# KyleKWKim/LLM-guided-Multimodal-MIL

Hardware: AMD Instinct MI355X
Metric: bags/sec fwd+bwd, N=1024 patches D=512 (higher is better)
Workload: dtype f32; 1 GPU; 32 bags/GPU x 1024 patches x 512 dims, image-only gated-attention MIL fwd+BCE+bwd+allreduce+Adam (BASELINE config 2; x1 GPUs = 32 bags); bags_per_gpu=32, patches=1024, dim=512, global_bags=32, parallelism=dp1, mode=train (dropout 0.5 on patches + 0.25 before the head, in-kernel masks), accum=1, batches_cycled=4, launch=eager

## Files before the change

llm-guided-multimodal-mil_amd/csrc/gate_reduce.h:

```cpp
#pragma once
#include "mil_common.h"
#define GR_NG 384
#define GR_NB 16

__device__ __forceinline__ unsigned short gp_bf16_bits(float v) { return __builtin_bit_cast(unsigned short, (__bf16)v); }
__device__ __forceinline__ float gp_bf16_val(unsigned short b) { return __uint_as_float(((unsigned)b) << 16); }
__device__ __forceinline__ void gp_split3(float v, unsigned short& p0, unsigned short& p1, unsigned short& p2) {
    p0 = gp_bf16_bits(v);
    float r = v - gp_bf16_val(p0);
    r = __builtin_isfinite(r) ? r : 0.f;
    p1 = gp_bf16_bits(r);
    p2 = gp_bf16_bits(r - gp_bf16_val(p1));
}
#define GP_SLICE_ELEMS (3 * 2 * GR_NG * 8)
__host__ __device__ __forceinline__ size_t gp_index(int q, int n, int k) {
    return (size_t)(k >> 4) * GP_SLICE_ELEMS + ((size_t)(q * 2 + ((k >> 3) & 1)) * GR_NG + n) * 8 + (k & 7);
}
__device__ __forceinline__ void gp_store4(unsigned short* __restrict__ Wp, int n, int k, const f32x4 v) {
    ushort4 o[3];
    gp_split3(v[0], o[0].x, o[1].x, o[2].x);
    gp_split3(v[1], o[0].y, o[1].y, o[2].y);
    gp_split3(v[2], o[0].z, o[1].z, o[2].z);
    gp_split3(v[3], o[0].w, o[1].w, o[2].w);
#pragma unroll
    for (int q = 0; q < 3; ++q) *reinterpret_cast<ushort4*>(Wp + gp_index(q, n, k)) = o[q];
}

struct HeadBwdArgs {
    const float* dz;
    const float* M;
    float* dWf;
    float* dbf;
    const float* loss_bag;
    float* loss_out;
    int B, L, C;
    int accumulate;
};
static __device__ __forceinline__ void head_bwd_params_block(const HeadBwdArgs& a, int blk, float (*red)[64],
                                                             const AdamFuse& ad) {
    const int nlb = (a.L + 63) / 64;
    const int lane = threadIdx.x & 63, g = threadIdx.x >> 6;
    if (blk < a.C * nlb) {
        const int c = blk / nlb, j = (blk % nlb) * 64 + lane;
        float v = 0.f;
        if (j < a.L)
            for (int b0 = g; b0 < a.B; b0 += 32) {
                float dzv[8], mv[8];
#pragma unroll
                for (int e = 0; e < 8; ++e) {
                    const int b = min(b0 + 4 * e, a.B - 1);
                    dzv[e] = a.dz[b * a.C + c];
                    mv[e] = a.M[(size_t)b * a.L + j];
                }
#pragma unroll
                for (int e = 0; e < 8; ++e) v = b0 + 4 * e < a.B ? fmaf(dzv[e], mv[e], v) : v;
            }
        red[g][lane] = v;
        __syncthreads();
        if (g == 0 && j < a.L) {
            float* o = a.dWf + (size_t)c * a.L + j;
            float t = red[0][lane] + red[1][lane] + red[2][lane] + red[3][lane];
            if (a.accumulate) t += *o;
            *o = t;
            adam_fused(ad, o, t);
        }
    } else {
        if ((int)threadIdx.x < a.C) {
            const int c = threadIdx.x;
            float v = 0.f;
            for (int b0 = 0; b0 < a.B; b0 += 16) {
                float u[16];
#pragma unroll
                for (int e = 0; e < 16; ++e) u[e] = a.dz[min(b0 + e, a.B - 1) * a.C + c];
#pragma unroll
                for (int e = 0; e < 16; ++e) v += b0 + e < a.B ? u[e] : 0.f;
            }
            if (a.accumulate) v += a.dbf[c];
            a.dbf[c] = v;
            adam_fused(ad, a.dbf + c, v);
        }
        if (a.loss_bag != nullptr && g == 1) {
            float v = 0.f;
            for (int b = lane; b < a.B; b += 64) v += a.loss_bag[b];
            v = wave_allsum(v);
            if (lane == 0) a.loss_out[0] = a.accumulate ? a.loss_out[0] + v : v;
        }
    }
}

static __global__ __launch_bounds__(256) void k_gate_bwd_reduce(const float* __restrict__ part, const float* __restrict__ pbias,
                                                                int S, int SB, int L, float* __restrict__ dWv, float* __restrict__ dbv,
                                                                float* __restrict__ dWu, float* __restrict__ dbu,
                                                                float* __restrict__ dw, float* __restrict__ db, int accumulate,
                                                                float wscale, int head_first = 1 << 30,
                                                                HeadBwdArgs head = HeadBwdArgs{}, AdamFuse ad_in = AdamFuse{},
// ... 126 lines not shown
```

llm-guided-multimodal-mil_amd/csrc/gated_pool.hip:

```cpp
#include "mil_internal.h"
#include "philox.h"
#include "gate_reduce.h"
#include <type_traits>

#define GF_TM 128
#define GF_BK 32
#define GF_NG 384

typedef __attribute__((address_space(3))) void lds_void;
__device__ __forceinline__ unsigned bitmask1(unsigned m, int b) { return (unsigned)__builtin_amdgcn_sbfe((int)m, b, 1); }
__device__ __forceinline__ float keep_if(float v, unsigned m, int b) {
    return __uint_as_float(__float_as_uint(v) & bitmask1(m, b));
}
template <bool DROP>
__global__ __launch_bounds__(512) void k_gate_fwd(const float* __restrict__ x, const float* __restrict__ Wv,
                                                       const float* __restrict__ bv, const float* __restrict__ Wu,
                                                       const float* __restrict__ bu, const float* __restrict__ wvec,
                                                       const float* __restrict__ battn, float* __restrict__ scores,
                                                       float* __restrict__ gates, int R, int L,
                                                       const uint32_t* __restrict__ xbits, float xscale) {
    __shared__ __attribute__((aligned(16))) float smem[2 * (GF_TM + GF_NG) * 32];
    float* xs = smem;
    float* ws = smem + 2 * GF_TM * 32;
    const int tid = threadIdx.x, lane = tid & 63, wave = tid >> 6;
// ... 1090 lines not shown
#pragma unroll
                    for (int i = 0; i < 16; ++i) acc[a][b][i] += fold[((a * 2 + b) * 16 + i) * 64 + lane];
        }
    }

    {
        __syncthreads();
        if (grp == 0) {
            float* tw = smem + wave * (64 * 64);
#pragma unroll
            for (int a = 0; a < 2; ++a)
#pragma unroll
                for (int b = 0; b < 2; ++b)
#pragma unroll
                    for (int i = 0; i < 16; ++i) tw[(32 * a + mfma32_row(i, h)) * 64 + 32 * b + r] = acc[a][b][i];
            float* pt = part + ((size_t)s * GF_NG + 128 * m + 64 * wi) * L + j0 + 64 * wj;
            const int c4 = lane & 15, rr = lane >> 4;
#pragma unroll
            for (int pass = 0; pass < 16; ++pass) {
                const int row = 4 * pass + rr;
                const f32x4 v = *reinterpret_cast<const f32x4*>(tw + row * 64 + 4 * c4);
                *reinterpret_cast<f32x4*>(pt + (size_t)row * L + 4 * c4) = v;
            }
        }
    }
#else
    {
        __syncthreads();
        float* tw = smem + wave * (64 * 64);
#pragma unroll
        for (int a = 0; a < 2; ++a)
#pragma unroll
            for (int b = 0; b < 2; ++b)
#pragma unroll
                for (int i = 0; i < 16; ++i) tw[(32 * a + mfma32_row(i, h)) * 64 + 32 * b + r] = acc[a][b][i];
        if (KG == 2) __syncthreads();
        float* pt = part + ((size_t)s * GF_NG + 128 * m + 64 * wi) * L + j0 + 64 * wj;
        const int c4 = lane & 15, rr = lane >> 4;
        const float* t0 = smem_all + wave * (64 * 64);
        const float* t1 = smem_all + (2 * 2 * GB_BKR * 128) + wave * (64 * 64);
        constexpr int NP = 16 / KG;
#pragma unroll
        for (int pass = 0; pass < NP; ++pass) {
            const int row = 4 * (pass + NP * grp) + rr;
            f32x4 v = *reinterpret_cast<const f32x4*>(t0 + row * 64 + 4 * c4);
            if (KG == 2) v += *reinterpret_cast<const f32x4*>(t1 + row * 64 + 4 * c4);
            *reinterpret_cast<f32x4*>(pt + (size_t)row * L + 4 * c4) = v;
        }
    }
#endif

    if (jt == 0) {
        float* redf = smem_all;
        const int arow_all = arow + 16 * grp;
        __syncthreads();
#pragma unroll
        for (int e = 0; e < 4; ++e) {
            redf[(arow_all * 3 + 0) * 64 + 4 * ad4 + e] = acc_bv[e];
            redf[(arow_all * 3 + 1) * 64 + 4 * ad4 + e] = acc_bu[e];
            redf[(arow_all * 3 + 2) * 64 + 4 * ad4 + e] = acc_w[e];
        }
        __syncthreads();
        if (grp == 0 && tid < 192) {
            const int which = tid / 64, d = tid % 64;
            float v = 0.f;
#pragma unroll
            for (int g = 0; g < 16 * KG; ++g) v += redf[(g * 3 + which) * 64 + d];
            pbias[((size_t)s * 4 + which) * 192 + 64 * m + d] = v;
        }
        if (m == 0) {
            __syncthreads();
            redf[threadIdx.x] = acc_ds;
            __syncthreads();
            if (threadIdx.x == 0) {
                float v = 0.f;
                for (int g = 0; g < 256 * KG; g += 16) v += redf[g];
                pbias[((size_t)s * 4 + 3) * 192] = v;
            }
        }
    }
}



template <bool DROP>
__global__ __launch_bounds__(512) void k_gate_bwd_dw2(const float* __restrict__ x, const float* __restrict__ gates,
                                                      const float* __restrict__ ds, const float* __restrict__ wvec,
                                                      float* __restrict__ part, float* __restrict__ pbias, int R, int L,
                                                      int KC, int NJ, const uint32_t* __restrict__ xbits,
                                                      const int32_t* __restrict__ rows_dev) {
    __shared__ __attribute__((aligned(16))) float smem_all[2 * 2 * 2 * GB_BKR * 128];
    if (rows_dev != nullptr) R = min(R, __builtin_amdgcn_readfirstlane(rows_dev[0]));
    const int grp = __builtin_amdgcn_readfirstlane((int)(threadIdx.x >> 8));
    float* smem = smem_all + grp * (2 * 2 * GB_BKR * 128);
    const int tid = threadIdx.x & 255, lane = tid & 63, wave = tid >> 6;
    const int wi = wave >> 1, wj = wave & 1;
    const int r = lane & 31, h = lane >> 5;
    int bid = blockIdx.x;
    {
        const int nwg = gridDim.x, q = nwg >> 3, rem = nwg & 7, xcd = bid & 7;
        bid = (xcd < rem ? xcd * (q + 1) : rem * (q + 1) + (xcd - rem) * q) + (bid >> 3);
    }
    const int jt = bid % NJ, m = (bid / NJ) % 3, s = bid / (3 * NJ);
    const int j0 = jt * 128;
    const int cbeg = min(s * KC, R), cend = min(R, cbeg + KC);
    const int half = ((cend - cbeg + 2 * GB_BKR - 1) / (2 * GB_BKR)) * GB_BKR;
    const int rbeg = min(cend, cbeg + grp * half), rend = min(cend, rbeg + half);
    const int nloop = (min(half, cend - cbeg) + GB_BKR - 1) / GB_BKR;

    const int xrow = tid >> 5, xc4 = tid & 31;
    const int arow = tid >> 4, ad4 = tid & 15;
    const int LW = L >> 5;
    int vx[4], vm[4], vg[2], vd[2];
#pragma unroll
    for (int i = 0; i < 4; ++i) {
        vx[i] = ((xrow + 8 * i) * L + j0 + 4 * xc4) * 4;
        vm[i] = ((xrow + 8 * i) * LW + ((j0 + 4 * xc4) >> 5)) * 4;
    }
#pragma unroll
    for (int i = 0; i < 2; ++i) {
        vg[i] = ((arow + 16 * i) * GF_NG + 64 * m + 4 * ad4) * 4;
        vd[i] = (arow + 16 * i) * 4;
    }
    const f32x4 w4 = *reinterpret_cast<const f32x4*>(wvec + 64 * m + 4 * ad4);
    auto blkpos = [](int c) { return (c & 31) | ((c & 32) << 1) | ((c & 64) >> 1); };
    float* const ab = smem;
    float* const xb = smem + 2 * GB_BKR * 128;
    float* const xw = xb + xrow * 128 + blkpos(4 * xc4);
    float* const aw = ab + arow * 128 + blkpos(4 * ad4);
    const float* const ap = ab + h * 128 + 32 * wi + r;
    const float* const bp = xb + h * 128 + 32 * wj + r;

    u32x4_t rx[4], rv[2], ru[2];
    unsigned rm[4] = {0, 0, 0, 0};
    float rds[2];
    f32x4 rt[2];
    f32x4 acc_bv = {0, 0, 0, 0}, acc_bu = {0, 0, 0, 0}, acc_w = {0, 0, 0, 0};
    float acc_ds = 0.f;

    auto x_srd = [&](int row0) {
        return __builtin_amdgcn_make_buffer_rsrc((void*)(x + (size_t)row0 * L), 0, max(rend - row0, 0) * L * 4, MIL_SRD_FLAGS);
    };
    auto g_srd = [&](int row0) {
        return __builtin_amdgcn_make_buffer_rsrc((void*)(gates + (size_t)row0 * GF_NG), 0, max(rend - row0, 0) * GF_NG * 4,
                                                 MIL_SRD_FLAGS);
    };
    auto d_srd = [&](int row0) {
        return __builtin_amdgcn_make_buffer_rsrc((void*)(ds + row0), 0, max(rend - row0, 0) * 4, MIL_SRD_FLAGS);
    };
    auto m_srd = [&](int row0) {
        return __builtin_amdgcn_make_buffer_rsrc((void*)(xbits + (size_t)row0 * LW), 0, max(rend - row0, 0) * LW * 4,
                                                 MIL_SRD_FLAGS);
    };
    auto xload = [&](int i, int row0) {
        rx[i] = __builtin_amdgcn_raw_buffer_load_b128(x_srd(row0), vx[i], 0, 0);
        if (DROP) rm[i] = __builtin_amdgcn_raw_buffer_load_b32(m_srd(row0), vm[i], 0, 0);
    };
    auto aload = [&](int i, int row0) {
        const __amdgpu_buffer_rsrc_t g = g_srd(row0);
        rv[i] = __builtin_amdgcn_raw_buffer_load_b128(g, vg[i], 0, 0);
        ru[i] = __builtin_amdgcn_raw_buffer_load_b128(g, vg[i] + 192 * 4, 0, 0);
        rds[i] = __uint_as_float(__builtin_amdgcn_raw_buffer_load_b32(d_srd(row0), vd[i], 0, 0));
    };
    auto xwrite = [&](int i, int buf) {
        f32x4 v = __builtin_bit_cast(f32x4, rx[i]);
        if (DROP) {
// ... 13 lines not shown
    auto awrite_u = [&](int i, int buf, bool pub) {
        const f32x4 t = rt[i], u = __builtin_bit_cast(f32x4, ru[i]);
        const f32x4 pu = t - t * u;
        *reinterpret_cast<f32x4*>(aw + (buf * GB_BKR + 16 * i) * 128 + 32) = pu;
        if (pub) {
            const f32x4 v = __builtin_bit_cast(f32x4, rv[i]);
            acc_bv += (rds[i] * w4) * u - t * v;
            acc_bu += pu;
            acc_w += (rds[i] * v) * u;
            if (ad4 == 0) acc_ds += rds[i];
        }
    };

    f32x16 acc[2][2];
#pragma unroll
    for (int a = 0; a < 2; ++a)
#pragma unroll
        for (int b = 0; b < 2; ++b)
#pragma unroll
            for (int i = 0; i < 16; ++i) acc[a][b][i] = 0.f;

#pragma unroll
    for (int i = 0; i < 4; ++i) xload(i, rbeg);
#pragma unroll
    for (int i = 0; i < 2; ++i) aload(i, rbeg);
#pragma unroll
    for (int i = 0; i < 4; ++i) xwrite(i, 0);
#pragma unroll
    for (int i = 0; i < 2; ++i) { awrite_v(i, 0); awrite_u(i, 0, jt == 0); }
#pragma unroll
    for (int i = 0; i < 4; ++i) xload(i, rbeg + GB_BKR);
#pragma unroll
    for (int i = 0; i < 2; ++i) aload(i, rbeg + GB_BKR);
    __syncthreads();

    auto slice = [&](int sl, auto buf_c) {
        constexpr int buf = decltype(buf_c)::value;
        const int row2 = rbeg + (sl + 2) * GB_BKR;
        const bool pub = ((sl + 1) % NJ) == jt;
        const float* apb = ap + buf * GB_BKR * 128;
        const float* bpb = bp + buf * GB_BKR * 128;
        float fa[2][2], fb[2][2];
        fa[0][0] = apb[0]; fa[0][1] = apb[64]; fb[0][0] = bpb[0]; fb[0][1] = bpb[64];
#pragma unroll
        for (int ks = 0; ks < GB_BKR / 2; ++ks) {
            const int q = ks & 1;
            acc[0][0] = __builtin_amdgcn_mfma_f32_32x32x2f32(fa[q][0], fb[q][0], acc[0][0], 0, 0, 0);
            __builtin_amdgcn_sched_barrier(0);
            if (ks + 1 < GB_BKR / 2) {
                fa[q ^ 1][0] = apb[(ks + 1) * 256]; fa[q ^ 1][1] = apb[(ks + 1) * 256 + 64];
                fb[q ^ 1][0] = bpb[(ks + 1) * 256]; fb[q ^ 1][1] = bpb[(ks + 1) * 256 + 64];
            }
            __builtin_amdgcn_sched_barrier(0);
            acc[0][1] = __builtin_amdgcn_mfma_f32_32x32x2f32(fa[q][0], fb[q][1], acc[0][1], 0, 0, 0);
            __builtin_amdgcn_sched_barrier(0);
            if (ks >= 1 && ks <= 4) xwrite(ks - 1, buf ^ 1);
            if (ks == 5) awrite_v(0, buf ^ 1);
            if (ks == 6) awrite_u(0, buf ^ 1, pub);
            if (ks == 7) awrite_v(1, buf ^ 1);
            if (ks == 8) awrite_u(1, buf ^ 1, pub);
            __builtin_amdgcn_sched_barrier(0);
            acc[1][0] = __builtin_amdgcn_mfma_f32_32x32x2f32(fa[q][1], fb[q][0], acc[1][0], 0, 0, 0);
            __builtin_amdgcn_sched_barrier(0);
            if (ks >= 1 && ks <= 4) xload(ks - 1, row2);
            if (ks == 6) aload(0, row2);
            if (ks == 8) aload(1, row2);
            __builtin_amdgcn_sched_barrier(0);
            acc[1][1] = __builtin_amdgcn_mfma_f32_32x32x2f32(fa[q][1], fb[q][1], acc[1][1], 0, 0, 0);
            __builtin_amdgcn_sched_barrier(0);
        }
    };
    int sl = 0;
    for (; sl + 1 < nloop; sl += 2) {
        slice(sl, std::integral_constant<int, 0>{});
        __syncthreads();
        slice(sl + 1, std::integral_constant<int, 1>{});
        __syncthreads();
    }
    if (sl < nloop) {
        slice(sl, std::integral_constant<int, 0>{});
        __syncthreads();
    }

    {
        float* tw = smem + wave * (64 * 64);
#pragma unroll
        for (int a = 0; a < 2; ++a)
#pragma unroll
            for (int b = 0; b < 2; ++b)
#pragma unroll
                for (int i = 0; i < 16; ++i) tw[(32 * a + mfma32_row(i, h)) * 64 + 32 * b + r] = acc[a][b][i];
        __syncthreads();
        float* pt = part + ((size_t)s * GF_NG + 128 * m + 64 * wi) * L + j0 + 64 * wj;
        const int c4 = lane & 15, rr = lane >> 4;
        const float* t0 = smem_all + wave * (64 * 64);
        const float* t1 = smem_all + (2 * 2 * GB_BKR * 128) + wave * (64 * 64);
#pragma unroll
        for (int pass = 0; pass < 8; ++pass) {
            const int row = 4 * (pass + 8 * grp) + rr;
            const f32x4 v = *reinterpret_cast<const f32x4*>(t0 + row * 64 + 4 * c4) +
                            *reinterpret_cast<const f32x4*>(t1 + row * 64 + 4 * c4);
            *reinterpret_cast<f32x4*>(pt + (size_t)row * L + 4 * c4) = v;
        }
    }

    {
        float* redf = smem_all;
        const int arow_all = arow + 16 * grp;
        __syncthreads();
#pragma unroll
        for (int e = 0; e < 4; ++e) {
            redf[(arow_all * 3 + 0) * 64 + 4 * ad4 + e] = acc_bv[e];
            redf[(arow_all * 3 + 1) * 64 + 4 * ad4 + e] = acc_bu[e];
            redf[(arow_all * 3 + 2) * 64 + 4 * ad4 + e] = acc_w[e];
        }
        __syncthreads();
        float* pb = pbias + ((size_t)s * NJ + jt) * 4 * 192;
        if (threadIdx.x < 192) {
            const int which = threadIdx.x / 64, d = threadIdx.x % 64;
            float v = 0.f;
#pragma unroll
            for (int g = 0; g < 32; ++g) v += redf[(g * 3 + which) * 64 + d];
            pb[which * 192 + 64 * m + d] = v;
        }
        if (m == 0) {
            __syncthreads();
            redf[threadIdx.x] = acc_ds;
            __syncthreads();
            if (threadIdx.x == 0) {
                float v = 0.f;
                for (int g = 0; g < 512; g += 16) v += redf[g];
                pb[3 * 192] = v;
            }
        }
    }
}

#include "gate_reduce.h"

extern "C" int mil_abi_version(void) { return 8; }

#define GS_TM 32
#define GS_LS 36
#define GS_THREADS 768
template <bool DROP, int RT>
__global__ __launch_bounds__(GS_THREADS) void k_gate_fwd_r32(const float* __restrict__ x, const float* __restrict__ Wv,
                                                             const float* __restrict__ bv, const float* __restrict__ Wu,
                                                             const float* __restrict__ bu, const float* __restrict__ wvec,
                                                             const float* __restrict__ battn, float* __restrict__ scores,
                                                             float* __restrict__ gates, int R, int L,
                                                             const uint32_t* __restrict__ xbits, float xscale,
                                                             const int32_t* __restrict__ rows_dev) {
    constexpr int TM = GS_TM * RT;
    if (rows_dev != nullptr && (int)(blockIdx.x * TM) >= __builtin_amdgcn_readfirstlane(rows_dev[0])) return;
    __shared__ __attribute__((aligned(16))) float smem[2 * (TM + GF_NG) * GS_LS];
    float* xs = smem;
    float* ws = smem + 2 * TM * GS_LS;
    const int tid = threadIdx.x, lane = tid & 63, wave = tid >> 6;
    const int c = wave >> 1, isu = wave & 1;
    const int r = lane & 31, h = lane >> 5;
    const int row0 = blockIdx.x * TM;
    const float* wsrc[4];
    int wdst[4];
#pragma unroll
    for (int i = 0; i < 4; ++i) {
        const int id = tid + GS_THREADS * i, wrow = id >> 3, ch = id & 7;
        wsrc[i] = (wrow < 192 ? Wv + (size_t)wrow * L : Wu + (size_t)(wrow - 192) * L) + 4 * ch;
        wdst[i] = wrow * GS_LS + 4 * ch;
    }
    const int xrow = (tid % (256 * RT)) >> 3, xch = tid & 7;
    const float* xsrc = x + (size_t)min(row0 + xrow, R - 1) * L + 4 * xch;
    const uint32_t* msrc = DROP ? xbits + (size_t)min(row0 + xrow, R - 1) * (L / 32) : nullptr;
    const int xdst = xrow * GS_LS + 4 * xch;
    f32x4 wreg[2][4], xreg[2];
    unsigned mreg[2] = {0, 0};
    auto gload = [&](int set, int k0) {
#pragma unroll
        for (int i = 0; i < 4; ++i) wreg[set][i] = *reinterpret_cast<const f32x4*>(wsrc[i] + k0);
        xreg[set] = *reinterpret_cast<const f32x4*>(xsrc + k0);
        if (DROP) mreg[set] = msrc[k0 >> 5];
    };
    auto swrite = [&](int set, int buf) {
#pragma unroll
        for (int i = 0; i < 4; ++i) *reinterpret_cast<f32x4*>(ws + buf * GF_NG * GS_LS + wdst[i]) = wreg[set][i];
        if (tid < 256 * RT) {
            f32x4 v = xreg[set];
            if (DROP) {
                const unsigned m = mreg[set] >> (4 * xch);
#pragma unroll
                for (int e = 0; e < 4; ++e) v[e] = keep_if(v[e], m, e) * xscale;
            }
            *reinterpret_cast<f32x4*>(xs + buf * TM * GS_LS + xdst) = v;
        }
    };
    f32x16 acc[RT];
#pragma unroll
    for (int q = 0; q < RT; ++q)
#pragma unroll
        for (int i = 0; i < 16; ++i) acc[q][i] = 0.f;
    const int nslice = L / GF_BK;
    gload(0, 0);
    swrite(0, 0);
    gload(1, min(1, nslice - 1) * GF_BK);
    gload(0, min(2, nslice - 1) * GF_BK);
    __syncthreads();
    auto iteration = [&](int s, int set) {
        const int buf = s & 1;
        const float* xa = xs + buf * TM * GS_LS + r * GS_LS + 4 * h;
        const float* wb = ws + buf * GF_NG * GS_LS + (192 * isu + 32 * c + r) * GS_LS + 4 * h;
        f32x4 fa[RT][4], fb[4];
#pragma unroll
        for (int t = 0; t < 4; ++t) {
#pragma unroll
            for (int q = 0; q < RT; ++q) fa[q][t] = *reinterpret_cast<const f32x4*>(xa + q * GS_TM * GS_LS + 8 * t);
            fb[t] = *reinterpret_cast<const f32x4*>(wb + 8 * t);
        }
        swrite(set, buf ^ 1);
        gload(set, min(s + 3, nslice - 1) * GF_BK);
// ... 340 lines not shown
    MIL_CHECK_LAUNCH();
    return MIL_OK;
}

extern "C" int mil_attn_pool_partial_h(const float* x, const float* scores, const int32_t* tile_map, int T, int L,
                                       float* partials, const float* Wf, int C, float* hrow, const uint32_t* xbits,
                                       float xscale, const uint32_t* mbits, float mscale, void* stream) {
    if (!x || !scores || !tile_map || !partials || !Wf || !hrow) return MIL_EINVAL;
    if (L <= 0 || (L % 256) != 0 || L > 1024 || T < 0 || C <= 0 || C > 4) return MIL_EINVAL;
    return launch_pool_partial(x, scores, tile_map, T, L, partials, Wf, C, hrow, (hipStream_t)stream, xbits, xscale, mbits,
                               mscale);
}

extern "C" int mil_attn_pool_bwd_from_h(const float* scores, const float* lse, const float* hrow, const float* dz,
                                        const float* cdot, const int32_t* tile_map, int T, int C, float* ds, void* stream) {
    if (!scores || !lse || !hrow || !dz || !cdot || !tile_map || !ds || T < 0 || C <= 0 || C > 4) return MIL_EINVAL;
    if (T == 0) return MIL_OK;
    hipLaunchKernelGGL(k_pool_ds_from_h, dim3((T + 7) / 8), dim3(256), 0, (hipStream_t)stream, scores, lse, hrow, dz, cdot,
                       tile_map, T, C, ds);
    MIL_CHECK_LAUNCH();
    return MIL_OK;
}

extern "C" int mil_attn_pool_partial(const float* x, const float* scores, const int32_t* tile_map, int T, int L,
                                     float* partials, const uint32_t* xbits, float xscale, void* stream) {
    if (!x || !scores || !tile_map || !partials) return MIL_EINVAL;
    if (L <= 0 || (L % 256) != 0 || L > 1024 || T < 0) return MIL_EINVAL;
    return launch_pool_partial(x, scores, tile_map, T, L, partials, nullptr, 0, nullptr, (hipStream_t)stream, xbits, xscale);
}

extern "C" int mil_attn_pool_fwd(const float* x, const float* scores, const int32_t* tile_map,
                                 const int32_t* bag_tile_off, int T, int B, int L, float* partials, float* M,
                                 float* lse, const uint32_t* xbits, float xscale, void* stream) {
    if (!x || !scores || !tile_map || !bag_tile_off || !partials || !M || !lse) return MIL_EINVAL;
    if (L <= 0 || (L % 256) != 0 || L > 1024 || B < 0 || T < 0) return MIL_EINVAL;
    hipStream_t st = (hipStream_t)stream;
    const int rc = launch_pool_partial(x, scores, tile_map, T, L, partials, nullptr, 0, nullptr, st, xbits, xscale);
    if (rc != MIL_OK) return rc;
    if (B > 0) {
        hipLaunchKernelGGL(k_pool_merge, dim3(B, L / 128), dim3(256), 0, st, partials, bag_tile_off, M, lse, L, T);
        MIL_CHECK_LAUNCH();
    }
    return MIL_OK;
}

extern "C" int mil_attn_pool_bwd(const float* x, const float* scores, const float* lse, const float* dM,
                                 const float* cdot, const int32_t* tile_map, int T, int L, float* ds, float* dx,
                                 const uint32_t* xbits, float xscale, void* stream) {
    if (!x || !scores || !lse || !dM || !cdot || !tile_map || !ds) return MIL_EINVAL;
    if (L <= 0 || (L % 256) != 0 || L > 1024 || T < 0) return MIL_EINVAL;
    if (T == 0) return MIL_OK;
    hipStream_t st = (hipStream_t)stream;
    switch (L / 256) {
        case 1: hipLaunchKernelGGL(k_pool_bwd_ds<1>, dim3(T), dim3(256), 0, st, x, scores, lse, dM, cdot, tile_map, ds, dx, L, xbits, xscale); break;
        case 2: hipLaunchKernelGGL(k_pool_bwd_ds<2>, dim3(T), dim3(256), 0, st, x, scores, lse, dM, cdot, tile_map, ds, dx, L, xbits, xscale); break;
        case 3: hipLaunchKernelGGL(k_pool_bwd_ds<3>, dim3(T), dim3(256), 0, st, x, scores, lse, dM, cdot, tile_map, ds, dx, L, xbits, xscale); break;
        default: hipLaunchKernelGGL(k_pool_bwd_ds<4>, dim3(T), dim3(256), 0, st, x, scores, lse, dM, cdot, tile_map, ds, dx, L, xbits, xscale); break;
    }
    MIL_CHECK_LAUNCH();
    return MIL_OK;
}

template <bool XB16>
static void launch_gate_bwd_dw(const void* x, const float* gates, const float* ds, const float* w, float* part, float* pbias,
                               int R, int L, int kc, int NJ, int S, int kg, const uint32_t* xbits, hipStream_t st,
                               const int32_t* rows_dev = nullptr) {
    const dim3 grid(S * 3 * NJ);
    if (kg == 2) {
        if (xbits) hipLaunchKernelGGL((k_gate_bwd_dw<XB16, 2, true>), grid, dim3(512), 0, st, x, gates, ds, w, part, pbias, R, L, kc, NJ, xbits, rows_dev);
        else hipLaunchKernelGGL((k_gate_bwd_dw<XB16, 2, false>), grid, dim3(512), 0, st, x, gates, ds, w, part, pbias, R, L, kc, NJ, xbits, rows_dev);
    } else {
        if (xbits) hipLaunchKernelGGL((k_gate_bwd_dw<XB16, 1, true>), grid, dim3(256), 0, st, x, gates, ds, w, part, pbias, R, L, kc, NJ, xbits, rows_dev);
        else hipLaunchKernelGGL((k_gate_bwd_dw<XB16, 1, false>), grid, dim3(256), 0, st, x, gates, ds, w, part, pbias, R, L, kc, NJ, xbits, rows_dev);
    }
}

static inline size_t gate_bwd_ws_floats(int S, int L) { return (size_t)S * GF_NG * L + (size_t)S * (L / 128) * 4 * 192; }

extern "C" size_t mil_gate_bwd_workspace_floats(int R, int L) {
    if (R <= 0 || L <= 0 || (L % 128) != 0) return 0;
    return gate_bwd_ws_floats(gate_dw_plan(R, L, MIL_NUM_CU).S, L);
}

static int gate_bwd_partials_impl(const float* x, const float* gates, const float* ds, const float* w, int R, int L,
                                  int D, float* workspace, size_t workspace_floats, const uint32_t* xbits,
                                  const int32_t* rows_dev, void* stream) {
    if (!x || !gates || !ds || !w || !workspace) return MIL_EINVAL;
    if (D != MIL_GATE_D || L <= 0 || (L % 128) != 0 || R <= 0) return MIL_EINVAL;
    const GateDwPlan p = gate_dw_plan(R, L, MIL_NUM_CU);
    const int S = p.S, kc = p.kc, NJ = L / 128;
    if (workspace_floats < gate_bwd_ws_floats(S, L)) return MIL_ENOSPC;
    float* pb = workspace + (size_t)S * GF_NG * L;
    if (p.dw == MIL_ROUTE_DW2) {
        if (xbits)
            hipLaunchKernelGGL(k_gate_bwd_dw2<true>, dim3(S * 3 * NJ), dim3(512), 0, (hipStream_t)stream, x, gates, ds, w, workspace, pb,
                               R, L, kc, NJ, xbits, rows_dev);
        else
            hipLaunchKernelGGL(k_gate_bwd_dw2<false>, dim3(S * 3 * NJ), dim3(512), 0, (hipStream_t)stream, x, gates, ds, w, workspace, pb,
                               R, L, kc, NJ, xbits, rows_dev);
        MIL_CHECK_LAUNCH();
        return MIL_OK;
    }
    launch_gate_bwd_dw<false>((const void*)x, gates, ds, w, workspace, pb, R, L, kc, NJ, S, p.dw == MIL_ROUTE_DW_KG2 ? 2 : 1, xbits,
                              (hipStream_t)stream, rows_dev);
    MIL_CHECK_LAUNCH();
    return MIL_OK;
}

extern "C" int mil_gate_bwd_partials(const float* x, const float* gates, const float* ds, const float* w, int R, int L,
                                     int D, float* workspace, size_t workspace_floats, const uint32_t* xbits,
                                     void* stream) {
    return gate_bwd_partials_impl(x, gates, ds, w, R, L, D, workspace, workspace_floats, xbits, nullptr, stream);
}
extern "C" int mil_gate_bwd_partials_rows(const float* x, const float* gates, const float* ds, const float* w, int R, int L,
                                          int D, float* workspace, size_t workspace_floats, const uint32_t* xbits,
                                          const int32_t* rows_dev, void* stream) {
    return gate_bwd_partials_impl(x, gates, ds, w, R, L, D, workspace, workspace_floats, xbits, rows_dev, stream);
}

static int gate_bwd_fold(const float* workspace, int R, int L, float* dWv, float* dbv, float* dWu, float* dbu, float* dw, float* db,
                         int accumulate, float wscale, void* stream, const HeadBwdArgs* head = nullptr,
                         const AdamFuse* ad = nullptr, uint16_t* Wp = nullptr) {
    const GateDwPlan p = gate_dw_plan(R, L, MIL_NUM_CU);
    return launch_gate_bwd_reduce(workspace, workspace + (size_t)p.S * GF_NG * L, p.S, p.dw == MIL_ROUTE_DW2 ? p.S * (L / 128) : p.S,
                                  L, dWv, dbv, dWu, dbu, dw, db, accumulate, wscale, (hipStream_t)stream, head, ad, nullptr,
                                  nullptr, Wp);
}

extern "C" int mil_gate_bwd_reduce(const float* workspace, int R, int L, float* dWv, float* dbv, float* dWu, float* dbu,
                                   float* dw, float* db, int accumulate, float xscale, void* stream) {
    if (!workspace || !dWv || !dbv || !dWu || !dbu || !dw || !db) return MIL_EINVAL;
    if (L <= 0 || (L % 128) != 0 || R <= 0) return MIL_EINVAL;
    return gate_bwd_fold(workspace, R, L, dWv, dbv, dWu, dbu, dw, db, accumulate, xscale, stream);
}

extern "C" int mil_gate_bwd_params_head(const float* x, const float* gates, const float* ds, const float* w, int R, int L,
                                        int D, float* workspace, size_t workspace_floats, float* dWv, float* dbv,
                                        float* dWu, float* dbu, float* dw, float* db, int accumulate, const float* dz,
                                        const float* M, float* dWf, float* dbf, int B, int C, const float* loss_bag,
                                        float* loss_out, const uint32_t* xbits, float xscale, void* stream) {
    if (!dWv || !dbv || !dWu || !dbu || !dw || !db || !dz || !M || !dWf || !dbf) return MIL_EINVAL;
    if (B <= 0 || C <= 0 || C > 32 || (loss_bag && !loss_out)) return MIL_EINVAL;
    const int rc = mil_gate_bwd_partials(x, gates, ds, w, R, L, D, workspace, workspace_floats, xbits, stream);
    if (rc != MIL_OK) return rc;
    const HeadBwdArgs head{dz, M, dWf, dbf, loss_bag, loss_out, B, L, C, accumulate};
    return gate_bwd_fold(workspace, R, L, dWv, dbv, dWu, dbu, dw, db, accumulate, xbits ? xscale : 1.0f, stream, &head);
}

extern "C" int mil_gate_bwd_reduce_head(const float* workspace, int R, int L, float* dWv, float* dbv, float* dWu, float* dbu,
                                        float* dw, float* db, int accumulate, float xscale, const float* dz, const float* M,
                                        float* dWf, float* dbf, int B, int C, const float* loss_bag, float* loss_out,
                                        void* stream) {
    if (!workspace || !dWv || !dbv || !dWu || !dbu || !dw || !db || !dz || !M || !dWf || !dbf) return MIL_EINVAL;
    if (L <= 0 || (L % 128) != 0 || R <= 0 || B <= 0 || C <= 0 || C > 32 || (loss_bag && !loss_out)) return MIL_EINVAL;
    const HeadBwdArgs head{dz, M, dWf, dbf, loss_bag, loss_out, B, L, C, accumulate};
    return gate_bwd_fold(workspace, R, L, dWv, dbv, dWu, dbu, dw, db, accumulate, xscale, stream, &head);
}

extern "C" int mil_gate_bwd_reduce_head_adam(const float* workspace, int R, int L, float* dWv, float* dbv, float* dWu,
                                             float* dbu, float* dw, float* db, int accumulate, float xscale, const float* dz,
                                             const float* M, float* dWf, float* dbf, int B, int C, const float* loss_bag,
                                             float* loss_out, float* param_flat, const float* grad_flat, size_t n_param,
                                             float* exp_avg, float* exp_avg_sq, int step, float lr, float beta1, float beta2,
                                             float eps, float weight_decay, float grad_scale, void* stream) {
    return gate_bwd_reduce_head_adam_impl(workspace, R, L, dWv, dbv, dWu, dbu, dw, db, accumulate, xscale, dz, M, dWf, dbf, B, C,
                                          loss_bag, loss_out, param_flat, grad_flat, n_param, exp_avg, exp_avg_sq, step, nullptr,
                                          lr, nullptr, beta1, beta2, eps, weight_decay, grad_scale, stream);
}

int gate_bwd_reduce_head_adam_impl(const float* workspace, int R, int L, float* dWv, float* dbv, float* dWu, float* dbu,
                                   float* dw, float* db, int accumulate, float xscale, const float* dz, const float* M,
                                   float* dWf, float* dbf, int B, int C, const float* loss_bag, float* loss_out,
                                   float* param_flat, const float* grad_flat, size_t n_param, float* exp_avg,
                                   float* exp_avg_sq, int step, const int* step_dev, float lr, const float* lr_dev, float beta1,
                                   float beta2, float eps, float weight_decay, float grad_scale, void* stream, int* done,
// ... 316 lines not shown
```

llm-guided-multimodal-mil_amd/csrc/gated_pool_bf16.hip:

```cpp
#include <stdlib.h>

#include "mil_internal.h"
#include "gate_reduce.h"

typedef __bf16 bf16x8 __attribute__((ext_vector_type(8)));
typedef unsigned short u16x8 __attribute__((ext_vector_type(8)));
typedef unsigned short u16;

__device__ __forceinline__ float bf16_to_f32(u16 v) { return __uint_as_float(((unsigned)v) << 16); }

__device__ __forceinline__ u16x8 keep_bf16x8(const u16x8 v, unsigned bits8) {
    typedef unsigned int u32x4k __attribute__((ext_vector_type(4)));
    u32x4k d = __builtin_bit_cast(u32x4k, v);
#pragma unroll
    for (int e = 0; e < 4; ++e) {
        const unsigned m2 = (bits8 >> (2 * e)) & 3u;
        const unsigned y = (m2 | (m2 << 15)) & 0x00010001u;
        d[e] &= (y << 16) - y;
    }
    return __builtin_bit_cast(u16x8, d);
}
__device__ __forceinline__ u16x8 keep_bf16x8_b(const u16x8 v, unsigned bits8) {
    typedef unsigned int u32x4k __attribute__((ext_vector_type(4)));
    u32x4k d = __builtin_bit_cast(u32x4k, v);
// ... 645 lines not shown
            head_row(c, wf);
#pragma unroll
            for (int i = 0; i < MIL_POOL_TILE / 4; ++i) {
                float d = 0.f;
#pragma unroll
                for (int q = 0; q < NQ; ++q)
#pragma unroll
                    for (int e = 0; e < 8; ++e) d += bf16_to_f32(v[i][q][e]) * wf[q][e];
                d = wave_allsum(d);
                const int rr = wave + 4 * i;
                if (lane == 0 && rr < nrows_) hrow[(size_t)(row0 + rr) * C + c] = d;
            }
        }
    }
    if (wave > 0) {
#pragma unroll
        for (int q = 0; q < NQ; ++q)
#pragma unroll
            for (int e = 0; e < 8; ++e) red[((wave - 1) * NQ + q) * 512 + 8 * lane + e] = acc[q][e];
    }
    __syncthreads();
    if (wave == 0) {
        float* out = partials + (size_t)t * L;
#pragma unroll
        for (int q = 0; q < NQ; ++q)
#pragma unroll
            for (int e = 0; e < 8; ++e) {
                float s = acc[q][e];
#pragma unroll
                for (int w = 0; w < 3; ++w) s += red[(w * NQ + q) * 512 + 8 * lane + e];
                out[512 * q + 8 * lane + e] = s;
            }
        if (lane == 0) {
            float* ml = partials + (size_t)gridDim.x * L + 2 * t;
            ml[0] = ml_lds[0];
            ml[1] = ml_lds[1];
        }
    }
}

template <int NQ>
__global__ __launch_bounds__(256) void k_pool_bwd_ds_bf16(const u16* __restrict__ x, const float* __restrict__ scores,
                                                          const float* __restrict__ lse, const float* __restrict__ dM,
                                                          const float* __restrict__ cdot,
                                                          const int32_t* __restrict__ tile_map, float* __restrict__ ds,
                                                          int L, const uint32_t* __restrict__ xbits, float xscale) {
    const int tid = threadIdx.x, lane = tid & 63, wave = tid >> 6;
    const int t = blockIdx.x;
    const int bag = tile_map[4 * t], row0 = tile_map[4 * t + 1], nrows = tile_map[4 * t + 2];
    float g[NQ][8];
#pragma unroll
    for (int q = 0; q < NQ; ++q)
#pragma unroll
        for (int e = 0; e < 8; ++e) g[q][e] = dM[(size_t)bag * L + 512 * q + 8 * lane + e];
    const float lse_b = lse[bag], c_b = cdot[bag];
    u16x8 v[MIL_POOL_TILE / 4][NQ];
    float sc[MIL_POOL_TILE / 4];
#pragma unroll
    for (int i = 0; i < MIL_POOL_TILE / 4; ++i) {
        const size_t row = (size_t)(row0 + min(wave + 4 * i, nrows - 1));
        const u16* xr = x + row * L + 8 * lane;
#pragma unroll
        for (int q = 0; q < NQ; ++q) v[i][q] = *reinterpret_cast<const u16x8*>(xr + 512 * q);
        if (xbits != nullptr) {
            const uint32_t* mr = xbits + row * (L >> 5) + (lane >> 2);
#pragma unroll
            for (int q = 0; q < NQ; ++q) v[i][q] = keep_bf16x8(v[i][q], mr[16 * q] >> (8 * (lane & 3)));
        }
        sc[i] = scores[row];
    }
#pragma unroll
    for (int i = 0; i < MIL_POOL_TILE / 4; ++i) {
        const int rr = wave + 4 * i;
        float dot = 0.f;
#pragma unroll
        for (int q = 0; q < NQ; ++q)
#pragma unroll
            for (int e = 0; e < 8; ++e) dot += bf16_to_f32(v[i][q][e]) * g[q][e];
        dot = wave_allsum(dot);
        if (rr < nrows && lane == 0) ds[row0 + rr] = expf(sc[i] - lse_b) * (dot * xscale - c_b);
    }
}

#define WB_S 160
typedef short s16x4 __attribute__((ext_vector_type(4)));
typedef __attribute__((address_space(3))) s16x4 lds_s16x4;

__device__ __forceinline__ u16x8 tr_frag(const u16* img, int row, int col) {
    const s16x4 lo = __builtin_amdgcn_ds_read_tr16_b64_v4i16((lds_s16x4*)(img + row * WB_S + col));
    const s16x4 hi = __builtin_amdgcn_ds_read_tr16_b64_v4i16((lds_s16x4*)(img + (row + 4) * WB_S + col));
    u16x8 f;
    f[0] = lo[0]; f[1] = lo[1]; f[2] = lo[2]; f[3] = lo[3];
    f[4] = hi[0]; f[5] = hi[1]; f[6] = hi[2]; f[7] = hi[3];
    return f;
}

__device__ __forceinline__ ushort4 pack_bf16x4(const f32x4 v) {
    ushort4 o;
    o.x = __builtin_bit_cast(u16, (__bf16)v[0]);
    o.y = __builtin_bit_cast(u16, (__bf16)v[1]);
    o.z = __builtin_bit_cast(u16, (__bf16)v[2]);
    o.w = __builtin_bit_cast(u16, (__bf16)v[3]);
    return o;
}

#define WB_BKR 64
#if !defined(WB_SETS)
#define WB_SETS 1
#endif
template <bool DROP>
__global__ __launch_bounds__(256) __attribute__((amdgpu_waves_per_eu(1, 1))) void k_gate_bwd_dw_bf16(const u16* __restrict__ x, const u16* __restrict__ gates,
                                                          const float* __restrict__ ds, const float* __restrict__ wvec,
                                                          float* __restrict__ part, float* __restrict__ pbias, int R, int L,
                                                          int KC, int NJ, const uint32_t* __restrict__ xbits) {
    __shared__ __attribute__((aligned(16))) u16 smem[2 * (WB_BKR * WB_S + WB_BKR * 2 * WB_S)];
    constexpr int ASZ = WB_BKR * WB_S, BSZ = WB_BKR * 2 * WB_S;
    u16* ab = smem;
    u16* xb = smem + 2 * ASZ;
    const int tid = threadIdx.x, lane = tid & 63, wave = tid >> 6;
    const int wi = wave >> 1, wj = wave & 1;
    const int h = lane >> 5;
    const int tq = (lane & 15) >> 2, tp = lane & 3, tg = (lane >> 4) & 1;
    int bid = blockIdx.x;
    {
        const int nwg = gridDim.x, q = nwg >> 3, rem = nwg & 7, xcd = bid & 7;
        bid = (xcd < rem ? xcd * (q + 1) : rem * (q + 1) + (xcd - rem) * q) + (bid >> 3);
    }
    const int jt = bid % NJ, m = (bid / NJ) % 3, s = bid / (3 * NJ);
    const int j0 = jt * 256;
    const int rbeg = s * KC, rend = min(R, rbeg + KC);
    const int nslice = (rend - rbeg + WB_BKR - 1) / WB_BKR;

    const int xrow = tid >> 5, xc = tid & 31;
    const int arow = tid >> 4, ad4 = tid & 15;
    const f32x4 w4 = *reinterpret_cast<const f32x4*>(wvec + 64 * m + 4 * ad4);
    u16x8 rx[WB_SETS][8];
    ushort4 hv[WB_SETS][4], hu[WB_SETS][4];
    float rds[WB_SETS][4], rmask[WB_SETS][4];
    f32x4 acc_bv = {0, 0, 0, 0}, acc_bu = {0, 0, 0, 0}, acc_w = {0, 0, 0, 0};
    float acc_ds = 0.f;

    unsigned rxm[WB_SETS][DROP ? 8 : 1];
    auto xload = [&](int z, int i, int rs) {
        const int gr = min(rs + xrow + 8 * i, rend - 1);
#if !defined(WB_ABL_NOX)
        rx[z][i] = *reinterpret_cast<const u16x8*>(x + (size_t)gr * L + j0 + 8 * xc);
#else
        asm volatile("" : "+v"(rx[z][i]) : "v"(gr));
#endif
        if (DROP) rxm[z][i] = xbits[(size_t)gr * (L >> 5) + ((j0 + 8 * xc) >> 5)];
    };
    auto xwrite = [&](int z, int i, int buf) {
        u16* dst = xb + buf * BSZ + (xc >> 4) * ASZ + (xrow + 8 * i) * WB_S + 8 * (xc & 15);
#if !defined(WB_ABL_NOXW)
        *reinterpret_cast<u16x8*>(dst) = DROP ? keep_bf16x8_b(rx[z][i], rxm[z][i] >> (8 * (xc & 3))) : rx[z][i];
#else
        asm volatile("" ::"v"(rx[z][i]), "v"(dst));
#endif
    };
    auto aload = [&](int z, int i, int rs, bool live) {
        const int gr = rs + arow + 16 * i;
        const int gc = min(gr, rend - 1);
        const u16* gp = gates + (size_t)gc * HB_NG + 64 * m + 4 * ad4;
#if !defined(WB_ABL_NOG)
        hv[z][i] = *reinterpret_cast<const ushort4*>(gp);
        hu[z][i] = *reinterpret_cast<const ushort4*>(gp + 192);
        rds[z][i] = ds[gc];
#else
        asm volatile("" : "+v"(hv[z][i]), "+v"(hu[z][i]), "+v"(rds[z][i]) : "v"(gp));
#endif
        rmask[z][i] = (live && gr < rend) ? 1.f : 0.f;
    };
    auto awrite = [&](int z, int i, int buf) {
#if defined(WB_ABL_NOAW)
        asm volatile("" ::"v"(hv[z][i]), "v"(hu[z][i]), "v"(rds[z][i]), "v"(buf));
        return;
#endif
        const f32x4 v = {bf16_to_f32(hv[z][i].x), bf16_to_f32(hv[z][i].y), bf16_to_f32(hv[z][i].z), bf16_to_f32(hv[z][i].w)};
// ... 532 lines not shown
```

Measured before the change: 153,100 bags/s.

## Add bf16x3-split MFMA path for gate backward weight-gradient kernel

Adds a new dW2 kernel that splits each fp32 operand of x and the gate-derived factors into three bf16 pieces, stages them in LDS and computes the product with 32x32x16 bf16 MFMAs. It uses six cross-piece products per slice, dropping the smallest terms, instead of the slow fp32 32x32x2 MFMA. The new kernel double-buffers with register prefetch interleaved between MFMAs. It is enabled by default via an environment switch. It trades exact fp32 accumulation for a near-fp32 emulation and adds split/convert ALU work and LDS traffic. The tile store and bias-sum epilogue are factored into shared helpers, and tr_frag moves into a common header.

```diff
diff --git a/llm-guided-multimodal-mil_amd/csrc/gate_reduce.h b/llm-guided-multimodal-mil_amd/csrc/gate_reduce.h
--- a/llm-guided-multimodal-mil_amd/csrc/gate_reduce.h
+++ b/llm-guided-multimodal-mil_amd/csrc/gate_reduce.h
@@ -11,6 +11,18 @@
     r = __builtin_isfinite(r) ? r : 0.f;
     p1 = gp_bf16_bits(r);
     p2 = gp_bf16_bits(r - gp_bf16_val(p1));
+}
+#define WB_S 160
+typedef short s16x4 __attribute__((ext_vector_type(4)));
+typedef __attribute__((address_space(3))) s16x4 lds_s16x4;
+typedef unsigned short gp_u16x8 __attribute__((ext_vector_type(8)));
+__device__ __forceinline__ gp_u16x8 tr_frag(const unsigned short* img, int row, int col) {
+    const s16x4 lo = __builtin_amdgcn_ds_read_tr16_b64_v4i16((lds_s16x4*)(img + row * WB_S + col));
+    const s16x4 hi = __builtin_amdgcn_ds_read_tr16_b64_v4i16((lds_s16x4*)(img + (row + 4) * WB_S + col));
+    gp_u16x8 f;
+    f[0] = lo[0]; f[1] = lo[1]; f[2] = lo[2]; f[3] = lo[3];
+    f[4] = hi[0]; f[5] = hi[1]; f[6] = hi[2]; f[7] = hi[3];
+    return f;
 }
 #define GP_SLICE_ELEMS (3 * 2 * GR_NG * 8)
 __host__ __device__ __forceinline__ size_t gp_index(int q, int n, int k) {
diff --git a/llm-guided-multimodal-mil_amd/csrc/gated_pool.hip b/llm-guided-multimodal-mil_amd/csrc/gated_pool.hip
--- a/llm-guided-multimodal-mil_amd/csrc/gated_pool.hip
+++ b/llm-guided-multimodal-mil_amd/csrc/gated_pool.hip
@@ -1196,6 +1196,61 @@
 }
 
 
+__device__ __forceinline__ void dw2_store_tile(float* smem_all, const f32x16 (&acc)[2][2], float* __restrict__ part, int s, int m,
+                                               int L, int j0, int grp, int wave, int lane) {
+    const int wi = wave >> 1, wj = wave & 1, r = lane & 31, h = lane >> 5;
+    float* tw = smem_all + grp * (2 * 2 * GB_BKR * 128) + wave * (64 * 64);
+#pragma unroll
+    for (int a = 0; a < 2; ++a)
+#pragma unroll
+        for (int b = 0; b < 2; ++b)
+#pragma unroll
+            for (int i = 0; i < 16; ++i) tw[(32 * a + mfma32_row(i, h)) * 64 + 32 * b + r] = acc[a][b][i];
+    __syncthreads();
+    float* pt = part + ((size_t)s * GF_NG + 128 * m + 64 * wi) * L + j0 + 64 * wj;
+    const int c4 = lane & 15, rr = lane >> 4;
+    const float* t0 = smem_all + wave * (64 * 64);
+    const float* t1 = smem_all + (2 * 2 * GB_BKR * 128) + wave * (64 * 64);
+#pragma unroll
+    for (int pass = 0; pass < 8; ++pass) {
+        const int row = 4 * (pass + 8 * grp) + rr;
+        const f32x4 v = *reinterpret_cast<const f32x4*>(t0 + row * 64 + 4 * c4) +
+                        *reinterpret_cast<const f32x4*>(t1 + row * 64 + 4 * c4);
+        *reinterpret_cast<f32x4*>(pt + (size_t)row * L + 4 * c4) = v;
+    }
+}
+__device__ __forceinline__ void dw2_publish_sums(float* smem_all, float* __restrict__ pbias, int s, int NJ, int jt, int m,
+                                                 int arow_all, int ad4, const f32x4 acc_bv, const f32x4 acc_bu,
+                                                 const f32x4 acc_w, float acc_ds) {
+    float* redf = smem_all;
+    __syncthreads();
+#pragma unroll
+    for (int e = 0; e < 4; ++e) {
+        redf[(arow_all * 3 + 0) * 64 + 4 * ad4 + e] = acc_bv[e];
+        redf[(arow_all * 3 + 1) * 64 + 4 * ad4 + e] = acc_bu[e];
+        redf[(arow_all * 3 + 2) * 64 + 4 * ad4 + e] = acc_w[e];
+    }
+    __syncthreads();
+    float* pb = pbias + ((size_t)s * NJ + jt) * 4 * 192;
+    if (threadIdx.x < 192) {
+        const int which = threadIdx.x / 64, d = threadIdx.x % 64;
+        float v = 0.f;
+#pragma unroll
+        for (int g = 0; g < 32; ++g) v += redf[(g * 3 + which) * 64 + d];
+        pb[which * 192 + 64 * m + d] = v;
+    }
+    if (m == 0) {
+        __syncthreads();
+        redf[threadIdx.x] = acc_ds;
+        __syncthreads();
+        if (threadIdx.x == 0) {
+            float v = 0.f;
+            for (int g = 0; g < 512; g += 16) v += redf[g];
+            pb[3 * 192] = v;
+        }
+    }
+}
+
 
 template <bool DROP>
 __global__ __launch_bounds__(512) void k_gate_bwd_dw2(const float* __restrict__ x, const float* __restrict__ gates,
@@ -1375,58 +1430,189 @@
         __syncthreads();
     }
 
+    dw2_store_tile(smem_all, acc, part, s, m, L, j0, grp, wave, lane);
+    dw2_publish_sums(smem_all, pbias, s, NJ, jt, m, arow + 16 * grp, ad4, acc_bv, acc_bu, acc_w, acc_ds);
+}
+
+#define GQ_PSZ (GB_BKR * WB_S)
+#define GQ_BUF (6 * GQ_PSZ)
+template <bool DROP>
+__global__ __launch_bounds__(512) void k_gate_bwd_dw2_pieces(const float* __restrict__ x, const float* __restrict__ gates,
+                                                             const float* __restrict__ ds, const float* __restrict__ wvec,
+                                                             float* __restrict__ part, float* __restrict__ pbias, int R, int L,
+                                                             int KC, int NJ, const uint32_t* __restrict__ xbits,
+                                                             const int32_t* __restrict__ rows_dev) {
+    __shared__ __attribute__((aligned(16))) float smem_all[2 * 2 * 2 * GB_BKR * 128];
+    static_assert(2 * GQ_BUF * 2 <= (int)sizeof(smem_all), "stages exceed the LDS image");
+    unsigned short* const img = reinterpret_cast<unsigned short*>(smem_all);
+    if (rows_dev != nullptr) R = min(R, __builtin_amdgcn_readfirstlane(rows_dev[0]));
+    const int grp = __builtin_amdgcn_readfirstlane((int)(threadIdx.x >> 8));
+    const int T = threadIdx.x, tid = T & 255, lane = tid & 63, wave = tid >> 6;
+    const int wi = wave >> 1, wj = wave & 1;
+    const int h = lane >> 5;
+    const int tq = (lane & 15) >> 2, tp = lane & 3, tg = (lane >> 4) & 1;
+    int bid = blockIdx.x;
     {
-        float* tw = smem + wave * (64 * 64);
-#pragma unroll
-        for (int a = 0; a < 2; ++a)
-#pragma unroll
-            for (int b = 0; b < 2; ++b)
-#pragma unroll
-                for (int i = 0; i < 16; ++i) tw[(32 * a + mfma32_row(i, h)) * 64 + 32 * b + r] = acc[a][b][i];
+        const int nwg = gridDim.x, q = nwg >> 3, rem = nwg & 7, xcd = bid & 7;
+        bid = (xcd < rem ? xcd * (q + 1) : rem * (q + 1) + (xcd - rem) * q) + (bid >> 3);
+    }
+    const int jt = bid % NJ, m = (bid / NJ) % 3, s = bid / (3 * NJ);
+    const int j0 = jt * 128;
+    const int rbeg = min(s * KC, R), rend = min(R, rbeg + KC);
+    const int nloop = (rend - rbeg + GB_BKR - 1) / GB_BKR;
+
+    const int xrow = T >> 5, xc4 = T & 31;
+    const int arow = T >> 4, ad4 = T & 15;
+    const int LW = L >> 5;
+    int vx[2], vm[2];
+#pragma unroll
+    for (int i = 0; i < 2; ++i) {
+        vx[i] = ((xrow + 16 * i) * L + j0 + 4 * xc4) * 4;
+        vm[i] = ((xrow + 16 * i) * LW + ((j0 + 4 * xc4) >> 5)) * 4;
+    }
+    const int vg = (arow * GF_NG + 64 * m + 4 * ad4) * 4, vd = arow * 4;
+    const f32x4 w4 = *reinterpret_cast<const f32x4*>(wvec + 64 * m + 4 * ad4);
+    unsigned short* const xw = img + 3 * GQ_PSZ + xrow * WB_S + 4 * xc4;
+    unsigned short* const aw = img + arow * WB_S + 4 * ad4;
+    const int frow = 16 * grp + 8 * h + tq;
+    const int acol = 64 * wi + 16 * tg + 4 * tp;
+    const int bcol = 64 * wj + 16 * tg + 4 * tp;
+
+    u32x4_t rx[2], rv, ru;
+    unsigned rm[2] = {0, 0};
+    float rds;
+    f32x4 rt;
+    f32x4 acc_bv = {0, 0, 0, 0}, acc_bu = {0, 0, 0, 0}, acc_w = {0, 0, 0, 0};
+    float acc_ds = 0.f;
+
+    auto xload = [&](int i, int row0) {
+        const int left = max(rend - row0, 0);
+        rx[i] = __builtin_amdgcn_raw_buffer_load_b128(
+            __builtin_amdgcn_make_buffer_rsrc((void*)(x + (size_t)row0 * L), 0, left * L * 4, MIL_SRD_FLAGS), vx[i], 0, 0);
+        if (DROP)
+            rm[i] = __builtin_amdgcn_raw_buffer_load_b32(
+                __builtin_amdgcn_make_buffer_rsrc((void*)(xbits + (size_t)row0 * LW), 0, left * LW * 4, MIL_SRD_FLAGS), vm[i], 0, 0);
+    };
+    auto aload = [&](int row0) {
+        const int left = max(rend - row0, 0);
+        const __amdgpu_buffer_rsrc_t g =
+            __builtin_amdgcn_make_buffer_rsrc((void*)(gates + (size_t)row0 * GF_NG), 0, left * GF_NG * 4, MIL_SRD_FLAGS);
+        rv = __builtin_amdgcn_raw_buffer_load_b128(g, vg, 0, 0);
+        ru = __builtin_amdgcn_raw_buffer_load_b128(g, vg + 192 * 4, 0, 0);
+        rds = __uint_as_float(__builtin_amdgcn_raw_buffer_load_b32(
+            __builtin_amdgcn_make_buffer_rsrc((void*)(ds + row0), 0, left * 4, MIL_SRD_FLAGS), vd, 0, 0));
+    };
+    auto put3 = [&](unsigned short* dst, const f32x4 v) {
+        ushort4 o[3];
+        gp_split3(v[0], o[0].x, o[1].x, o[2].x);
+        gp_split3(v[1], o[0].y, o[1].y, o[2].y);
+        gp_split3(v[2], o[0].z, o[1].z, o[2].z);
+        gp_split3(v[3], o[0].w, o[1].w, o[2].w);
+#pragma unroll
+        for (int q = 0; q < 3; ++q) *reinterpret_cast<ushort4*>(dst + q * GQ_PSZ) = o[q];
+    };
+    auto xwrite = [&](int i, int buf) {
+        f32x4 v = __builtin_bit_cast(f32x4, rx[i]);
+        if (DROP) {
+            const unsigned mm = rm[i] >> (4 * (xc4 & 7));
+#pragma unroll
+            for (int e = 0; e < 4; ++e) v[e] = keep_if(v[e], mm, e);
+        }
+        put3(xw + buf * GQ_BUF + 16 * i * WB_S, v);
+    };
+    auto awrite_v = [&](int buf) {
+        const f32x4 v = __builtin_bit_cast(f32x4, rv);
+        const f32x4 a = (rds * w4) * __builtin_bit_cast(f32x4, ru);
+        const f32x4 t = a * v;
+        rt = t;
+        put3(aw + buf * GQ_BUF, a - t * v);
+    };
+    auto awrite_u = [&](int buf, bool pub) {
+        const f32x4 t = rt, u = __builtin_bit_cast(f32x4, ru);
+        const f32x4 pu = t - t * u;
+        put3(aw + buf * GQ_BUF + 64, pu);
+        if (pub) {
+            const f32x4 v = __builtin_bit_cast(f32x4, rv);
+            acc_bv += (rds * w4) * u - t * v;
+            acc_bu += pu;
+            acc_w += (rds * v) * u;
+            if (ad4 == 0) acc_ds += rds;
+        }
+    };
+
+    f32x16 acc[2][2];
+#pragma unroll
+    for (int a = 0; a < 2; ++a)
+#pragma unroll
+        for (int b = 0; b < 2; ++b)
+#pragma unroll
+            for (int i = 0; i < 16; ++i) acc[a][b][i] = 0.f;
+
+    gp_u16x8 fa[2][3][2], fb[2][3][2];
+    auto frags = [&](auto set_c, int buf) {
+        constexpr int set = decltype(set_c)::value;
+        const unsigned short* ai = img + buf * GQ_BUF;
+#pragma unroll
+        for (int p = 2; p >= 0; --p) {
+#pragma unroll
+            for (int a = 0; a < 2; ++a) fa[set][p][a] = tr_frag(ai + p * GQ_PSZ, frow, acol + 32 * a);
+#pragma unroll
+            for (int b = 0; b < 2; ++b) fb[set][p][b] = tr_frag(ai + (3 + p) * GQ_PSZ, frow, bcol + 32 * b);
+        }
+    };
+
+    xload(0, rbeg); xload(1, rbeg); aload(rbeg);
+    xwrite(0, 0); xwrite(1, 0); awrite_v(0); awrite_u(0, jt == 0);
+    xload(0, rbeg + GB_BKR); xload(1, rbeg + GB_BKR); aload(rbeg + GB_BKR);
+    __syncthreads();
+    frags(std::integral_constant<int, 0>{}, 0);
+
+    auto slice = [&](int sl, auto set_c) {
+        constexpr int set = decltype(set_c)::value;
+        constexpr int TP[6] = {0, 1, 2, 0, 1, 0}, TQ[6] = {2, 1, 0, 1, 0, 0};
+        const int row2 = rbeg + (sl + 2) * GB_BKR;
+        const bool pub = ((sl + 1) % NJ) == jt;
+        auto mfma = [&](int t, int g) {
+            const int a = g >> 1, b = g & 1;
+            acc[a][b] = __builtin_amdgcn_mfma_f32_32x32x16_bf16(__builtin_bit_cast(gp_bf16x8, fa[set][TP[t]][a]),
+                                                                __builtin_bit_cast(gp_bf16x8, fb[set][TQ[t]][b]), acc[a][b], 0, 0, 0);
+        };
+#pragma unroll
+        for (int t = 0; t < 3; ++t)
+#pragma unroll
+            for (int g = 0; g < 4; ++g) {
+                mfma(t, g);
+                __builtin_amdgcn_sched_barrier(0);
+                switch (4 * t + g) {
+                    case 0: xwrite(0, set ^ 1); break;
+                    case 1: xload(0, row2); break;
+                    case 2: xwrite(1, set ^ 1); break;
+                    case 3: xload(1, row2); break;
+                    case 4: awrite_v(set ^ 1); break;
+                    case 5: awrite_u(set ^ 1, pub); break;
+                    case 6: aload(row2); break;
+                    default: break;
+                }
+                __builtin_amdgcn_sched_barrier(0);
+            }
         __syncthreads();
-        float* pt = part + ((size_t)s * GF_NG + 128 * m + 64 * wi) * L + j0 + 64 * wj;
-        const int c4 = lane & 15, rr = lane >> 4;
-        const float* t0 = smem_all + wave * (64 * 64);
-        const float* t1 = smem_all + (2 * 2 * GB_BKR * 128) + wave * (64 * 64);
-#pragma unroll
-        for (int pass = 0; pass < 8; ++pass) {
-            const int row = 4 * (pass + 8 * grp) + rr;
-            const f32x4 v = *reinterpret_cast<const f32x4*>(t0 + row * 64 + 4 * c4) +
-                            *reinterpret_cast<const f32x4*>(t1 + row * 64 + 4 * c4);
-            *reinterpret_cast<f32x4*>(pt + (size_t)row * L + 4 * c4) = v;
-        }
-    }
-
-    {
-        float* redf = smem_all;
-        const int arow_all = arow + 16 * grp;
-        __syncthreads();
-#pragma unroll
-        for (int e = 0; e < 4; ++e) {
-            redf[(arow_all * 3 + 0) * 64 + 4 * ad4 + e] = acc_bv[e];
-            redf[(arow_all * 3 + 1) * 64 + 4 * ad4 + e] = acc_bu[e];
-            redf[(arow_all * 3 + 2) * 64 + 4 * ad4 + e] = acc_w[e];
-        }
-        __syncthreads();
-        float* pb = pbias + ((size_t)s * NJ + jt) * 4 * 192;
-        if (threadIdx.x < 192) {
-            const int which = threadIdx.x / 64, d = threadIdx.x % 64;
-            float v = 0.f;
-#pragma unroll
-            for (int g = 0; g < 32; ++g) v += redf[(g * 3 + which) * 64 + d];
-            pb[which * 192 + 64 * m + d] = v;
-        }
-        if (m == 0) {
-            __syncthreads();
-            redf[threadIdx.x] = acc_ds;
-            __syncthreads();
-            if (threadIdx.x == 0) {
-                float v = 0.f;
-                for (int g = 0; g < 512; g += 16) v += redf[g];
-                pb[3 * 192] = v;
-            }
-        }
-    }
+        if (sl + 1 < nloop) frags(std::integral_constant<int, set ^ 1>{}, set ^ 1);
+        __builtin_amdgcn_sched_barrier(0);
+#pragma unroll
+        for (int t = 3; t < 6; ++t)
+#pragma unroll
+            for (int g = 0; g < 4; ++g) mfma(t, g);
+    };
+    int sl = 0;
+    for (; sl + 1 < nloop; sl += 2) {
+        slice(sl, std::integral_constant<int, 0>{});
+        slice(sl + 1, std::integral_constant<int, 1>{});
+    }
+    if (sl < nloop) slice(sl, std::integral_constant<int, 0>{});
+    __syncthreads();
+
+    dw2_store_tile(smem_all, acc, part, s, m, L, j0, grp, wave, lane);
+    dw2_publish_sums(smem_all, pbias, s, NJ, jt, m, arow, ad4, acc_bv, acc_bu, acc_w, acc_ds);
 }
 
 #include "gate_reduce.h"
@@ -1933,6 +2119,11 @@
     return gate_bwd_ws_floats(gate_dw_plan(R, L, MIL_NUM_CU).S, L);
 }
 
+static inline bool dw_pieces_on() {
+    const char* e = getenv("MIL_DW_PIECES");
+    return e == nullptr || atoi(e) != 0;
+}
+
 static int gate_bwd_partials_impl(const float* x, const float* gates, const float* ds, const float* w, int R, int L,
                                   int D, float* workspace, size_t workspace_floats, const uint32_t* xbits,
                                   const int32_t* rows_dev, void* stream) {
@@ -1942,6 +2133,16 @@
     const int S = p.S, kc = p.kc, NJ = L / 128;
     if (workspace_floats < gate_bwd_ws_floats(S, L)) return MIL_ENOSPC;
     float* pb = workspace + (size_t)S * GF_NG * L;
+    if (p.dw == MIL_ROUTE_DW2 && dw_pieces_on()) {
+        if (xbits)
+            hipLaunchKernelGGL(k_gate_bwd_dw2_pieces<true>, dim3(S * 3 * NJ), dim3(512), 0, (hipStream_t)stream, x, gates, ds, w, workspace, pb,
+                               R, L, kc, NJ, xbits, rows_dev);
+        else
+            hipLaunchKernelGGL(k_gate_bwd_dw2_pieces<false>, dim3(S * 3 * NJ), dim3(512), 0, (hipStream_t)stream, x, gates, ds, w, workspace, pb,
+                               R, L, kc, NJ, xbits, rows_dev);
+        MIL_CHECK_LAUNCH();
+        return MIL_OK;
+    }
     if (p.dw == MIL_ROUTE_DW2) {
         if (xbits)
             hipLaunchKernelGGL(k_gate_bwd_dw2<true>, dim3(S * 3 * NJ), dim3(512), 0, (hipStream_t)stream, x, gates, ds, w, workspace, pb,
diff --git a/llm-guided-multimodal-mil_amd/csrc/gated_pool_bf16.hip b/llm-guided-multimodal-mil_amd/csrc/gated_pool_bf16.hip
--- a/llm-guided-multimodal-mil_amd/csrc/gated_pool_bf16.hip
+++ b/llm-guided-multimodal-mil_amd/csrc/gated_pool_bf16.hip
@@ -751,18 +751,6 @@
     }
 }
 
-#define WB_S 160
-typedef short s16x4 __attribute__((ext_vector_type(4)));
-typedef __attribute__((address_space(3))) s16x4 lds_s16x4;
-
-__device__ __forceinline__ u16x8 tr_frag(const u16* img, int row, int col) {
-    const s16x4 lo = __builtin_amdgcn_ds_read_tr16_b64_v4i16((lds_s16x4*)(img + row * WB_S + col));
-    const s16x4 hi = __builtin_amdgcn_ds_read_tr16_b64_v4i16((lds_s16x4*)(img + (row + 4) * WB_S + col));
-    u16x8 f;
-    f[0] = lo[0]; f[1] = lo[1]; f[2] = lo[2]; f[3] = lo[3];
-    f[4] = hi[0]; f[5] = hi[1]; f[6] = hi[2]; f[7] = hi[3];
-    return f;
-}
 
 __device__ __forceinline__ ushort4 pack_bf16x4(const f32x4 v) {
     ushort4 o;
```

Result: faster. 178,200 bags/s, median of 6 (+16.4%).
